# caofff/GL-ABC-MCMC

Measured on AMD Instinct MI355X. Metric: MH accept-steps/sec (whole node) + ESJD, 65 536 chains, Mixture_set dim=2, higher is better.
Workload: dtype f32; 1 GPU; GLMCMC iSIR N=5 gf=0.9, Mixture_set eps=0.05 d=2 (BASELINE configs[1]); chains_per_gpu=65536, batch_size=5, history=True, math_mode=exact, lanes_per_chain=auto, parallelism=chains sharded over 1 GPU(s), no data-path collective

## Files before the change

gl-abc-mcmc_amd/csrc/glabc_device.h:

```cpp
#pragma once

#if !defined(__HIPCC_RTC__)
#include <hip/hip_runtime.h>
#include <stdint.h>
#endif

#include "../../include/glabc.h"
#include "../../include/glabc_numerics.h"

namespace glabc {

#define GLABC_DEV static __device__ __forceinline__

enum Algo { ALGO_GLMCMC = 0, ALGO_GLOBAL = 1 };

enum Variant { VAR_GENERIC = 0, VAR_GAUSS_UNIT = 1, VAR_TAPE = 2, VAR_GAMMA = 3, VAR_MIX = 4 };

template <int D>
struct DistArgs {
    int32_t kind;
    int32_t unit_scale;
    float c0;
    float p0[D], p1[D], p2[D];
    float p3[D];
// ... 256 lines not shown
        const double lp = glabc_gamma_log_pdf((double)g.p0[q], (double)g.p2[q], (double)g.p3[q], z);
#pragma unroll
        for (int r = 0; r < D; ++r) {
            if (r == q) {
                th[r] = (float)z;
                t[r] = lp;
            }
        }
    }
    lq = (float)aten_rowsum_f64<D>(t);
}

template <int D>
GLABC_DEV double mix_mode_term(const MixArgs<D>& m, int k, const double (&z)[D])
{
    double t[D];
#pragma unroll
    for (int q = 0; q < D; ++q) {
        const double e = (z[q] - m.loc[k][q]) * m.inv_scale[k][q];
        t[q] = e * e;
    }
    return glabc_mix_term(m.c0 + m.log_weight[k], aten_rowsum_f64<D>(t), m.sum_log_scale[k]);
}

template <int D>
GLABC_DEV double mix_log_prob(const MixArgs<D>& m, const double (&z)[D])
{
    const int K = m.n_modes;
    double mx = -__builtin_inf();
#pragma unroll 1
    for (int k = 0; k < K; ++k) {
        const double t = mix_mode_term<D>(m, k, z);
        mx = t > mx ? t : mx;
    }
    if (mx == -__builtin_inf() || mx == __builtin_inf()) mx = 0.0;
    double a0 = 0.0, a1 = 0.0, a2 = 0.0, a3 = 0.0, tail = 0.0;
#pragma unroll 1
    for (int k = 0; k < K; ++k) {
        const double e = glabc_exp(mix_mode_term<D>(m, k, z) - mx);
        if (k < 4) {
            a0 = k == 0 ? e : a0;
            a1 = k == 1 ? e : a1;
            a2 = k == 2 ? e : a2;
            a3 = k == 3 ? e : a3;
        } else if (K == 8) {
            a0 = k == 4 ? a0 + e : a0;
            a1 = k == 5 ? a1 + e : a1;
            a2 = k == 6 ? a2 + e : a2;
            a3 = k == 7 ? a3 + e : a3;
        } else {
            tail = tail + e;
        }
    }
    double s;
    if (K < 4) {
        s = a0;
        if (K > 1) s = s + a1;
        if (K > 2) s = s + a2;
    } else {
        s = (((tail + a0) + a1) + a2) + a3;
    }
    return mx + glabc_log(s);
}

template <int D>
GLABC_DEV float dist_mix_log_prob(const MixArgs<D>& m, const float (&z)[D])
{
    double zd[D];
#pragma unroll
    for (int q = 0; q < D; ++q) zd[q] = (double)z[q];
    return (float)mix_log_prob<D>(m, zd);
}

template <int D>
GLABC_DEV void mix_draw(const MixArgs<D>& m, double u, const float (&eps)[D], double (&z)[D])
{
    double sc[D], lc[D];
#pragma unroll
    for (int q = 0; q < D; ++q) {
        sc[q] = m.scale[0][q];
        lc[q] = m.loc[0][q];
    }
#pragma unroll 1
    for (int k = 1; k < m.n_modes; ++k) {
        const bool up = !(u < m.cum_weight[k - 1]);
#pragma unroll
        for (int q = 0; q < D; ++q) {
            sc[q] = up ? m.scale[k][q] : sc[q];
            lc[q] = up ? m.loc[k][q] : lc[q];
        }
    }
#pragma unroll
    for (int q = 0; q < D; ++q) z[q] = (double)eps[q] * sc[q] + lc[q];
}

template <int D>
GLABC_DEV void dist_mix_forward(const MixArgs<D>& m, uint32_t c0, uint32_t c1, uint32_t k0, uint32_t k1, uint32_t step, int j,
                                const float (&eps)[D], float (&th)[D], float& lq)
{
    const glabc_u32x4 w = glabc_philox4x32_10(c0, c1, step, GLABC_SLOT_MIX + (uint32_t)j, k0, k1);
    double z[D];
    mix_draw<D>(m, glabc_uniform_f64(w.v[0], w.v[1]), eps, z);
#pragma unroll
    for (int q = 0; q < D; ++q) th[q] = (float)z[q];
    lq = (float)mix_log_prob<D>(m, z);
}

template <int D, bool KNOWN_GAUSS_UNIT = false, bool GAMMA_OK = false>
GLABC_DEV float dist_log_prob(const DistArgs<D>& g, const float (&z)[D])
{
    if constexpr (GAMMA_OK) {
        if (g.kind == GLABC_DIST_GAMMA) return dist_log_prob_gamma<D>(g, z);
    }
    if (KNOWN_GAUSS_UNIT || g.kind == GLABC_DIST_DIAG_GAUSS) {
        float t[D];
        if (KNOWN_GAUSS_UNIT || g.unit_scale) {
#pragma unroll
            for (int j = 0; j < D; ++j) {
                float e = z[j] - g.p0[j];
                t[j] = 0.5f * (e * e);
            }
        } else {
#pragma unroll
            for (int j = 0; j < D; ++j) {
                float e = (z[j] - g.p0[j]) / g.p2[j];
                t[j] = g.p1[j] + 0.5f * (e * e);
            }
        }
        return g.c0 - aten_rowsum<D>(t);
    } else {
        bool out = false;
#pragma unroll
        for (int j = 0; j < D; ++j) out = out || (z[j] < g.p0[j]) || (z[j] > g.p1[j]);
        return out ? -__builtin_inff() : g.c0;
    }
}

template <int D, bool KNOWN_GAUSS_UNIT = false>
GLABC_DEV float dist_forward_log_p(const DistArgs<D>& g, const float (&noise)[D])
{
    if (KNOWN_GAUSS_UNIT || g.kind == GLABC_DIST_DIAG_GAUSS) {
        float t[D];
#pragma unroll
        for (int j = 0; j < D; ++j) {
            const float h = 0.5f * (noise[j] * noise[j]);
            t[j] = KNOWN_GAUSS_UNIT ? h : g.p1[j] + h;
        }
        return g.c0 - aten_rowsum<D>(t);
    }
    return g.c0;
}

GLABC_DEV float gk_tanhf(float x)
{
    const float e = glabc_expf_core(__builtin_fmaxf(-2.0f * __builtin_fabsf(x), -104.0f));
    const float r = (1.0f - e) / (1.0f + e);
    return x < 0.0f ? -r : r;
}

template <int N>
GLABC_DEV void sort_ascending(float (&v)[N])
{
#pragma unroll
    for (int pass = 0; pass < N; ++pass) {
#pragma unroll
        for (int i = pass & 1; i + 1 < N; i += 2) {
            const float lo = __builtin_fminf(v[i], v[i + 1]), hi = __builtin_fmaxf(v[i], v[i + 1]);
            v[i] = lo;
            v[i + 1] = hi;
        }
    }
}

#ifdef GLABC_USER_SIM
template <int YD> struct NoiseDim { static constexpr int value = GLABC_USER_NOISE_DIM; };
#else
template <int YD> struct NoiseDim { static constexpr int value = YD; };
#endif

template <int D, int YD>
GLABC_DEV void model_simulate(const StepArgs<D, YD>& a, const float (&theta)[D], const float (&eps)[NoiseDim<YD>::value],
                              float (&y)[YD])
{
#ifdef GLABC_USER_SIM
    glabc_user_simulate(theta, eps, y);
    return;
#else
    if constexpr (YD == D) {
        if (D < 4 || a.sim_kind == GLABC_SIM_ABS_GAUSS) {
#pragma unroll
            for (int j = 0; j < YD; ++j) {
                float noise = a.noise_loc[j] + a.noise_scale[j] * eps[j];
                y[j] = __builtin_fabsf(theta[j]) + noise;
            }
            return;
        }
    }
    if constexpr (D >= 4) {
#pragma unroll
        for (int j = 0; j < YD; ++j) {
            const float z = eps[j];
            const float t = gk_tanhf((theta[2] * z) * 0.5f);
            const float pw = glabc_expf(theta[3] * glabc_logf_normal(1.0f + z * z));
            y[j] = theta[0] + ((theta[1] * (1.0f + a.gk_c * t)) * pw) * z;
        }
        sort_ascending<YD>(y);
    }
#endif
}

template <int YD>
GLABC_DEV float model_discrepancy_rows(const float (&y)[YD], const float* y_obs)
{
#ifdef GLABC_USER_DISCREPANCY
    float yo[YD];
#pragma unroll
    for (int j = 0; j < YD; ++j) yo[j] = y_obs[j];
    return glabc_user_discrepancy(y, yo);
#else
    float t[YD];
#pragma unroll
    for (int j = 0; j < YD; ++j) {
        float d = y[j] - y_obs[j];
        t[j] = d * d;
    }
    return __builtin_sqrtf(aten_rowsum<YD>(t));
#endif
}

GLABC_DEV float model_log_kernel_of(float dis, float kern_scale, float kern_log_scale, float kern_c0)
{
#ifdef GLABC_USER_KERNEL
    (void)kern_log_scale;
    (void)kern_c0;
    return glabc_user_log_kernel(dis, kern_scale);
#else
    const float e = (dis - 0.0f) / kern_scale;
    return kern_c0 - (kern_log_scale + 0.5f * (e * e));
#endif
}

template <int D, int YD, bool LEAN_SQRT = false, bool FAST = false>
GLABC_DEV float model_log_kernel(const StepArgs<D, YD>& a, const float (&y)[YD])
{
#if defined(GLABC_USER_DISCREPANCY) || defined(GLABC_USER_KERNEL)
    return model_log_kernel_of(model_discrepancy_rows<YD>(y, a.y_obs), a.kern_scale, a.kern_log_scale, a.kern_c0);
#else
    float t[YD];
#pragma unroll
    for (int j = 0; j < YD; ++j) {
        float d = y[j] - a.y_obs[j];
        t[j] = d * d;
    }
    const float ss = aten_rowsum<YD>(t);
    if constexpr (FAST) {
        const float e = __builtin_amdgcn_sqrtf(ss) * __builtin_amdgcn_rcpf(a.kern_scale);
        return a.kern_c0 - (a.kern_log_scale + 0.5f * (e * e));
    }
    float dis = LEAN_SQRT ? glabc_sqrtf_normal(ss) : __builtin_sqrtf(ss);
    float e;
    if constexpr (LEAN_SQRT) {
        const float q = dis * a.kern_rinv;
        e = __builtin_fmaf(__builtin_fmaf(-q, a.kern_scale, dis), a.kern_rinv, q);
    } else {
        e = (dis - 0.0f) / a.kern_scale;
    }
    return a.kern_c0 - (a.kern_log_scale + 0.5f * (e * e));
#endif
}

template <int D, int YD, bool GU, bool GM>
GLABC_DEV float model_prior(const StepArgs<D, YD>& a, const float (&theta)[D])
{
#ifdef GLABC_USER_PRIOR
    return glabc_user_prior_log_prob(theta);
#else
    return dist_log_prob<D, GU, GM>(a.prior, theta);
#endif
}

struct Rng {
    uint32_t c0, c1, k0, k1;
};

GLABC_DEV void fast_normal_pair(uint32_t a, uint32_t b, float* z0, float* z1)
{
    const float u1 = glabc_uniform_pos_f32(a);
    const float rad = __builtin_amdgcn_sqrtf(-1.3862943611198906f * __builtin_amdgcn_logf(u1));
    const float u2 = glabc_uniform_f32(b);
    *z0 = rad * __builtin_amdgcn_cosf(u2);
    *z1 = rad * __builtin_amdgcn_sinf(u2);
}
GLABC_DEV float fast_expf(float x)
{
    const float t = x * 1.4426950408889634f;
    const bool tiny = t < -126.0f;
    const float r = __builtin_amdgcn_exp2f(tiny ? t + 64.0f : t);
    return tiny ? r * 0x1p-64f : r;
}
GLABC_DEV float fast_logf(float x) { return 0.6931471805599453f * __builtin_amdgcn_logf(x); }

#if defined(__HIPCC_RTC__)
constexpr bool kFastPassWeights = false;
#else
constexpr bool kFastPassWeights = true;
#endif
GLABC_DEV float isir_weight(float lw)
{
    const float v = glabc_expf(lw);
    return (v != v) ? 0.0f : v;
}
GLABC_DEV float isir_weight_approx(float lw)
{
    const float x = __builtin_fminf(__builtin_fmaxf(lw, -104.0f), 100.0f);
    const float t = __builtin_fmaf(x, 0x1.715476p+0f, 12582912.0f);
    const float k = t - 12582912.0f;
    float r = __builtin_fmaf(k, -0x1.62e4p-1f, x);
    r = __builtin_fmaf(k, -0x1.7f7d1cp-20f, r);
    return __builtin_ldexpf(__builtin_amdgcn_exp2f(r * 0x1.715476p+0f), (int)k);
}

template <int L, int SRC>
GLABC_DEV int group_bcast_i(int v)
{
    if constexpr (L == 1) {
        return v;
    } else if constexpr (L == 2) {
        constexpr int ctrl = SRC | (SRC << 2) | ((2 + SRC) << 4) | ((2 + SRC) << 6);
        return __builtin_amdgcn_mov_dpp(v, ctrl, 0xf, 0xf, true);
    } else {
        static_assert(L == 4, "lane groups are 1, 2 or 4 wide");
        constexpr int ctrl = SRC | (SRC << 2) | (SRC << 4) | (SRC << 6);
        return __builtin_amdgcn_mov_dpp(v, ctrl, 0xf, 0xf, true);
    }
}

template <int L, int SRC>
GLABC_DEV float group_bcast(float v)
{
    return __builtin_bit_cast(float, group_bcast_i<L, SRC>(__builtin_bit_cast(int, v)));
}

template <int L>
GLABC_DEV float group_get_dyn(float v, int src)
{
    if constexpr (L == 1) {
        return v;
    } else {
        const int lane = (int)(threadIdx.x & 63u);
        return __shfl(v, (lane & ~(L - 1)) | src, 64);
    }
}

template <int L, int K, int NL>
GLABC_DEV float gather_weight(const float (&wl)[NL])
{
    return group_bcast<L, (K - 1) % L>(wl[(K - 1) / L]);
}

template <int L, int N, int NL, int K = 1>
GLABC_DEV void gather_weights(const float (&wl)[NL], float (&w)[N + 1])
{
    if constexpr (K <= N) {
        w[K] = gather_weight<L, K, NL>(wl);
        gather_weights<L, N, NL, K + 1>(wl, w);
    }
}

template <int D, int YD = D>
struct Chain {
    float theta[D];
    float y[YD];
    float prior;
    float kern;
    float q;
    float log_w;
    float lw_cur;
    float w_cur;
    float gf;
    uint32_t flags;
    uint32_t n_moves;
};

template <int D, int YD, bool GAMMA_OK = false>
GLABC_DEV void refresh_cache(const StepArgs<D, YD>& a, Chain<D, YD>& c)
{
    c.prior = model_prior<D, YD, false, GAMMA_OK>(a, c.theta);
    c.kern = model_log_kernel<D, YD>(a, c.y);
    c.q = dist_log_prob<D, false, GAMMA_OK>(a.global, c.theta);
}

template <int ALGO, int D, int YD, int N, int L, int VAR>
GLABC_DEV bool chain_step(const typename KernelArgs<D, YD, VAR>::type& a, const Rng& rng, uint32_t step, int sub, Chain<D, YD>& c, int64_t tape_pos)
{
    constexpr bool GU = (VAR == VAR_GAUSS_UNIT);
    constexpr bool TAPE = (VAR == VAR_TAPE);
    constexpr bool GM = (VAR == VAR_GAMMA);
    constexpr bool MX = (VAR == VAR_MIX);
    static_assert(!TAPE || L == 1, "tape replay runs one lane per chain");
    static_assert(!GM || L == 1, "the Gamma variant runs one lane per chain");
    static_assert(!MX || L == 1, "the mixture variant runs one lane per chain");
    constexpr int NL = (N + L - 1) / L;
    constexpr int HEAD = L - 1;
    constexpr bool FREE_SLOT = (L > 1) && (N % L != 0) && (NL >= 2);
    constexpr int DP = D + (D & 1);
    constexpr int ND = NoiseDim<YD>::value;
    constexpr int M = DP + ND;
    constexpr int SPP = (M + 3) / 4;

    uint32_t hw[4];
    float log_u = 0.0f;
    bool is_global = false;
    auto take_head = [&]() {
        if constexpr (L > 1) {
#pragma unroll
            for (int q = 0; q < 4; ++q) hw[q] = (uint32_t)group_bcast_i<L, HEAD>((int)hw[q]);
        }
        const float ub = TAPE ? a.tape_u[2 * tape_pos] : glabc_uniform_f32(hw[0]);
        const float ua = TAPE ? a.tape_u[2 * tape_pos + 1] : glabc_uniform_f32(hw[1]);
        log_u = TAPE ? glabc_logf(ua) : ((ua == 0.0f) ? -__builtin_inff() : glabc_logf_normal(ua));
        is_global = ub < c.gf;
        if (ALGO == ALGO_GLMCMC && is_global) {
            if (c.flags & GLABC_FLAG_LOCAL) c.log_w = c.lw_cur;
            c.flags &= ~GLABC_FLAG_LOCAL;
        }
    };
    if constexpr (!FREE_SLOT) {
        if (L == 1 || sub == HEAD) {
            glabc_u32x4 h = glabc_philox4x32_10(rng.c0, rng.c1, step, 0u, rng.k0, rng.k1);
#pragma unroll
            for (int q = 0; q < 4; ++q) hw[q] = h.v[q];
        } else {
#pragma unroll
            for (int q = 0; q < 4; ++q) hw[q] = 0u;
        }
        take_head();
    }

    [[maybe_unused]] float* mix_stage = nullptr;
    if constexpr (MX) {
        static_assert(D <= 4, "the mixture variant is instantiated up to theta_dim 4");
        __shared__ float mix_lds[N * (D + 1) * 64];
        mix_stage = mix_lds + (threadIdx.x & 63u);
#pragma unroll 1
        for (int j = 0; j < N; ++j) {
            const glabc_u32x4 o = glabc_philox4x32_10(rng.c0, rng.c1, step, (uint32_t)(1 + j * SPP), rng.k0, rng.k1);
            float nj[4], ej[D], tm[D], lqm;
            glabc_normal_pair(o.v[0], o.v[1], &nj[0], &nj[1]);
            if constexpr (D > 2) glabc_normal_pair(o.v[2], o.v[3], &nj[2], &nj[3]);
#pragma unroll
            for (int q = 0; q < D; ++q) ej[q] = nj[q];
            dist_mix_forward<D>(mix_of(a), rng.c0, rng.c1, rng.k0, rng.k1, step, j, ej, tm, lqm);
#pragma unroll
            for (int q = 0; q < D; ++q) mix_stage[(j * (D + 1) + q) * 64] = tm[q];
            mix_stage[(j * (D + 1) + D) * 64] = lqm;
        }
    }

    float th[NL][D], yy[NL][YD], lw[NL], pr[NL], kk[NL], wl[NL];
    bool acc_mh = false;
    const bool g_uni = !GU && a.global.kind == GLABC_DIST_UNIFORM;
    const bool l_uni = !GU && a.local.kind == GLABC_DIST_UNIFORM;
#pragma unroll
    for (int rr = 0; rr < NL; ++rr) {
        const int r = FREE_SLOT ? (NL - 1 - rr) : rr;
        const int j = sub + L * r;
        const bool head_pass = FREE_SLOT && (r == NL - 1);
        const bool first = (r == 0) && (L == 1 || sub == 0);
        uint32_t w[4 * SPP];
#pragma unroll
        for (int b = 0; b < SPP; ++b) {
            uint32_t slot_id = (uint32_t)(1 + j * SPP + b);
            if (head_pass && b == 0) slot_id = (sub == HEAD) ? 0u : slot_id;
            glabc_u32x4 o = glabc_philox4x32_10(rng.c0, rng.c1, step, slot_id, rng.k0, rng.k1);
#pragma unroll
            for (int q = 0; q < 4; ++q) w[4 * b + q] = o.v[q];
        }
        if (head_pass) {
#pragma unroll
            for (int q = 0; q < 4; ++q) hw[q] = w[q];
            take_head();
        }
        const bool loc = first && !is_global;
        const bool uni = loc ? l_uni : g_uni;
        float nrm[2 * ((M + 1) / 2)], e[D], s[ND];
#pragma unroll
        for (int i = 0; 2 * i < M; ++i) glabc_normal_pair(w[2 * i], w[2 * i + 1], &nrm[2 * i], &nrm[2 * i + 1]);
#pragma unroll
        for (int i = 0; i < D; ++i) e[i] = (!GU && uni) ? glabc_uniform_f32(w[i]) : nrm[i];
#pragma unroll
        for (int i = 0; i < ND; ++i) s[i] = nrm[DP + i];
        if constexpr (TAPE) {
            const float* tz = a.tape_z + (tape_pos * a.tape_nprop + (j < a.tape_nprop ? j : 0)) * (D + YD);
#pragma unroll
            for (int i = 0; i < D; ++i) e[i] = tz[i];
#pragma unroll
            for (int i = 0; i < ND; ++i) s[i] = tz[D + i];
        }
#pragma unroll
        for (int q = 0; q < D; ++q) {
            const float p0 = loc ? a.local.p0[q] : a.global.p0[q];
            const float p2 = loc ? a.local.p2[q] : a.global.p2[q];
            const float t = p0 + p2 * e[q];
            th[r][q] = loc ? (t + c.theta[q]) : t;
        }
        float lq_gamma = 0.0f;
        const bool g_gam = GM && a.global.kind == GLABC_DIST_GAMMA;
        if constexpr (GM) {
            if (g_gam) {
                float tg[D];
                dist_gamma_forward<D>(a.global, rng.c0, rng.c1, rng.k0, rng.k1, step, j, tg, lq_gamma);
#pragma unroll
                for (int q = 0; q < D; ++q) th[r][q] = loc ? th[r][q] : tg[q];
            }
        }
        float lq_mix = 0.0f;
        if constexpr (MX) {
            lq_mix = mix_stage[(r * (D + 1) + D) * 64];
#pragma unroll
            for (int q = 0; q < D; ++q) th[r][q] = loc ? th[r][q] : mix_stage[(r * (D + 1) + q) * 64];
        }
        float lq;
        if constexpr (MX) {
            lq = lq_mix;
            if constexpr (ALGO == ALGO_GLMCMC) {
                if (loc) lq = dist_mix_log_prob<D>(mix_of(a), th[r]);
            }
        } else if constexpr (ALGO == ALGO_GLMCMC && GU) {
            float v[D];
#pragma unroll
            for (int q = 0; q < D; ++q) v[q] = loc ? (th[r][q] - a.global.p0[q]) : e[q];
            lq = dist_forward_log_p<D, GU>(a.global, v);
        } else if constexpr (ALGO == ALGO_GLMCMC) {
            lq = loc ? dist_log_prob<D, GU, GM>(a.global, th[r]) : (g_gam ? lq_gamma : dist_forward_log_p<D, GU>(a.global, e));
        } else {
            lq = g_gam ? lq_gamma : dist_forward_log_p<D, GU>(a.global, e);
        }
        model_simulate<D, YD>(a, th[r], s, yy[r]);
        pr[r] = model_prior<D, YD, GU, GM>(a, th[r]);
        kk[r] = model_log_kernel<D, YD, GU>(a, yy[r]);
        const float pk = pr[r] + kk[r];
        lw[r] = pk - lq;
        if (r == 0) {
            float log_acc;
            if (ALGO == ALGO_GLOBAL)
                log_acc = loc ? ((pk - c.prior) - c.kern)
                              : ((((pk + c.q) - lq) - c.prior) - c.kern);
            else
                log_acc = (pk - c.prior) - c.kern;
            acc_mh = log_u < log_acc;
        }
        if (ALGO == ALGO_GLMCMC)
            wl[r] = kFastPassWeights ? isir_weight_approx(lw[r]) : isir_weight(lw[r]);
    }

    int ind;
    if constexpr (ALGO == ALGO_GLMCMC) {
        float w[N + 1];
        w[0] = c.w_cur;
        gather_weights<L, N, NL>(wl, w);
        float tot = aten_rowsum<N + 1>(w);
        const double u_res = TAPE ? a.tape_r[tape_pos] : glabc_uniform_f64(hw[2], hw[3]);
        int ig = -1;
        bool sure = !a.exact_index;
        {
            const float rinv = __builtin_amdgcn_rcpf(tot);
            const float u32 = (float)u_res;
            float run = 0.0f;
#pragma unroll
            for (int k = 0; k <= N; ++k) {
                run += w[k] * rinv;
                const float gap = u32 - run;
                sure = sure && (__builtin_fabsf(gap) > 4e-6f);
                ig = (ig < 0 && gap < 0.0f) ? k : ig;
            }
            sure = sure && (run > 0.999f) && (run < 1.001f);
            if constexpr (kFastPassWeights) sure = sure && (tot >= 0x1p-100f) && (tot < 0x1p126f);
        }
        if (!sure) {
            if constexpr (kFastPassWeights) {
                float lwg[N + 1];
                gather_weights<L, N, NL>(lw, lwg);
#pragma unroll
                for (int k = 1; k <= N; ++k) w[k] = isir_weight(lwg[k]);
                tot = aten_rowsum<N + 1>(w);
            }
            ig = -1;
            double run = 0.0;
#pragma unroll
            for (int k = 0; k <= N; ++k) {
                run += (double)(w[k] / tot);
                ig = (ig < 0 && u_res < run) ? k : ig;
            }
        }
        ig = ig < 0 ? 0 : ig;
        const int il = group_bcast_i<L, 0>(acc_mh ? 1 : 0);
        ind = is_global ? ig : il;
    } else {
        ind = group_bcast_i<L, 0>(acc_mh ? 1 : 0);
    }

    const bool moved = ind > 0;
    if (__any(moved)) {
        const int owner = (ind - 1) & (L - 1);
        const int slot = (ind - 1) / L;
        constexpr bool CARRY_W = (ALGO == ALGO_GLMCMC) && !kFastPassWeights;
        float nt[D], ny[YD], nlw = lw[0], npr = pr[0], nkk = kk[0], nw = CARRY_W ? wl[0] : 0.0f;
#pragma unroll
// ... 58 lines not shown
```

gl-abc-mcmc_amd/csrc/glabc_geometry.h:

```cpp
#pragma once

#include "../../include/glabc.h"

namespace glabc {


constexpr int team_main_candidates(int n, int nw)
{
    const int t10 = (10 * n + 11) / nw - 11;
    const int na = (t10 + 5) / 10;
    return na < 1 ? 1 : (na > n - (nw - 1) ? n - (nw - 1) : na);
}
constexpr int team_helper_first(int n, int nw, int h)
{
    const int na = team_main_candidates(n, nw), nh = n - na, per = nh / (nw - 1), extra = nh % (nw - 1);
    return na + h * per + (h < extra ? h : extra);
}
constexpr bool team_split_ok(int n, int nw) { return n >= nw && team_main_candidates(n, nw) >= 1; }

constexpr int team_lds_bytes(int d, int yd, int n, int nw) { return 2 * (n - team_main_candidates(n, nw)) * (4 + d + yd) * 64 * 4; }
constexpr int TEAM_MAX_LDS = 40 * 1024;
constexpr bool team_config_ok(int d, int yd, int n, int nw)
{
    return n >= 2 && n <= GLABC_MAX_BATCH && team_split_ok(n, nw) && team_lds_bytes(d, yd, n, nw) <= TEAM_MAX_LDS;
}

constexpr int GLOBAL_TEAM_CHUNK = 8;
constexpr int global_team_lds_bytes(int d, int nd) { return 2 * GLOBAL_TEAM_CHUNK * (2 + d + 2 * ((nd + 1) / 2)) * 64 * 4; }


constexpr int WIDE_BLOCK = 256;
constexpr int WIDE_LANES[4] = {8, 16, 32, 64};
constexpr int wide_default_lanes(int n) { return n <= 64 ? 8 : n <= 128 ? 16 : n <= 256 ? 32 : 64; }
constexpr int wide_row_floats(int n) { return n + 1 + 32; }
constexpr int64_t wide_lds_bytes(int l, int n) { return (int64_t)4 * (WIDE_BLOCK / l) * wide_row_floats(n); }


constexpr int pick_lanes(int requested, int n_batch, int64_t n_chains)
{
    int lanes = requested;
    if (lanes <= 0) {
        const int64_t chip_lanes = 64 * 1024;
        lanes = 1;
        while (lanes < 4 && n_chains * lanes < chip_lanes) lanes *= 2;
    }
    if (lanes >= 4 && n_batch >= 3) return 4;
    if (lanes >= 2 && n_batch >= 2) return 2;
    return 1;
}

}
```

gl-abc-mcmc_amd/csrc/glabc_team.h:

```cpp
#pragma once

#include "glabc_device.h"
#include "glabc_geometry.h"

namespace glabc {

template <int D, int YD, int NH>
struct TeamCand {
    float wl[NH][64];
    float lw[NH][64];
    float pr[NH][64];
    float kk[NH][64];
    float th[NH][D][64];
    float yy[NH][YD][64];
};

template <int D, int YD, int VAR, bool FIRST, bool FAST = false>
GLABC_DEV void team_candidate(const StepArgs<D, YD>& a, const Rng& rng, uint32_t step, int j, bool loc, const Chain<D, YD>& c,
                              float (&th)[D], float (&yy)[YD], float& lw, float& pr, float& kk, float& wl, int64_t row = 0,
                              int n_prop = 0, bool dump = false)
{
    constexpr bool GU = (VAR == VAR_GAUSS_UNIT);
    constexpr bool GM = (VAR == VAR_GAMMA);
    constexpr int DP = D + (D & 1);
    constexpr int ND = NoiseDim<YD>::value;
    constexpr int M = DP + ND;
    constexpr int SPP = (M + 3) / 4;
    const bool g_uni = !GU && a.global.kind == GLABC_DIST_UNIFORM;
    const bool l_uni = !GU && a.local.kind == GLABC_DIST_UNIFORM;
    uint32_t w[4 * SPP];
#pragma unroll
    for (int b = 0; b < SPP; ++b) {
        glabc_u32x4 o = glabc_philox4x32_10(rng.c0, rng.c1, step, (uint32_t)(1 + j * SPP + b), rng.k0, rng.k1);
#pragma unroll
        for (int q = 0; q < 4; ++q) w[4 * b + q] = o.v[q];
    }
    const bool lc = FIRST && loc;
    const bool uni = lc ? l_uni : g_uni;
    float nrm[2 * ((M + 1) / 2)], e[D], s[ND];
#pragma unroll
    for (int i = 0; 2 * i < M; ++i) {
        if constexpr (FAST) fast_normal_pair(w[2 * i], w[2 * i + 1], &nrm[2 * i], &nrm[2 * i + 1]);
        else glabc_normal_pair(w[2 * i], w[2 * i + 1], &nrm[2 * i], &nrm[2 * i + 1]);
    }
#pragma unroll
    for (int i = 0; i < D; ++i) e[i] = (!GU && uni) ? glabc_uniform_f32(w[i]) : nrm[i];
#pragma unroll
    for (int i = 0; i < ND; ++i) s[i] = nrm[DP + i];
    if constexpr (FAST) {
        if (dump) {
            float* z = a.dump_z + (row * n_prop + j) * (D + ND);
#pragma unroll
            for (int i = 0; i < D; ++i) z[i] = e[i];
#pragma unroll
            for (int i = 0; i < ND; ++i) z[D + i] = s[i];
        }
    }
#pragma unroll
    for (int q = 0; q < D; ++q) {
        const float p0 = lc ? a.local.p0[q] : a.global.p0[q];
        const float p2 = lc ? a.local.p2[q] : a.global.p2[q];
        const float t = (GU && !FIRST) ? p0 + e[q] : p0 + p2 * e[q];
        th[q] = lc ? (t + c.theta[q]) : t;
    }
    float lq_gamma = 0.0f;
    const bool g_gam = GM && a.global.kind == GLABC_DIST_GAMMA;
    if constexpr (GM) {
        if (g_gam) {
            float tg[D];
            dist_gamma_forward<D>(a.global, rng.c0, rng.c1, rng.k0, rng.k1, step, j, tg, lq_gamma);
#pragma unroll
            for (int q = 0; q < D; ++q) th[q] = lc ? th[q] : tg[q];
        }
    }
    float lq;
    if constexpr (GU) {
        float v[D];
#pragma unroll
        for (int q = 0; q < D; ++q) v[q] = lc ? (th[q] - a.global.p0[q]) : e[q];
        lq = dist_forward_log_p<D, GU>(a.global, v);
    } else {
        lq = lc ? dist_log_prob<D, GU, GM>(a.global, th) : (g_gam ? lq_gamma : dist_forward_log_p<D, GU>(a.global, e));
    }
    model_simulate<D, YD>(a, th, s, yy);
    pr = model_prior<D, YD, GU, GM>(a, th);
    kk = model_log_kernel<D, YD, GU, FAST>(a, yy);
    lw = (pr + kk) - lq;
    if constexpr (FAST) {
        const float v = fast_expf(lw);
        wl = (v != v) ? 0.0f : v;
    } else {
        wl = kFastPassWeights ? isir_weight_approx(lw) : isir_weight(lw);
    }
}

template <int D, int YD, int N, int VAR, int NA, int LO, int HI, bool FAST>
GLABC_DEV void team_helper(const StepArgs<D, YD>& a, const Rng& rng, int lane, TeamCand<D, YD, N - NA> (&buf)[2], int64_t chain, bool valid)
{
    Chain<D, YD> none;
#pragma unroll 1
    for (int t = 0; t < a.n_steps; ++t) {
        const uint32_t step = a.step0 + (uint32_t)t;
        TeamCand<D, YD, N - NA>& o = buf[t & 1];
#pragma unroll
        for (int j = LO; j < HI; ++j) {
            float th[D], yy[YD], lw, pr, kk, wl;
            team_candidate<D, YD, VAR, false, FAST>(a, rng, step, j, false, none, th, yy, lw, pr, kk, wl,
                                                    chain * (int64_t)a.n_steps + t, N, FAST && valid && a.dump_z != nullptr);
            o.wl[j - NA][lane] = wl;
            o.lw[j - NA][lane] = lw;
            o.pr[j - NA][lane] = pr;
            o.kk[j - NA][lane] = kk;
#pragma unroll
            for (int q = 0; q < D; ++q) o.th[j - NA][q][lane] = th[q];
#pragma unroll
            for (int q = 0; q < YD; ++q) o.yy[j - NA][q][lane] = yy[q];
        }
        __syncthreads();
    }
}

template <int D, int YD, int N, int VAR, int NW, bool FAST = false>
__global__ void __launch_bounds__(64 * NW) __attribute__((amdgpu_waves_per_eu(NW))) team_sampler_kernel(const StepArgs<D, YD> a, int prio)
{
    constexpr bool GU = (VAR == VAR_GAUSS_UNIT);
    constexpr bool GM = (VAR == VAR_GAMMA);
    static_assert(NW >= 2 && NW <= 4 && team_split_ok(N, NW), "team of two to four wavefronts, at least one candidate each");
    constexpr int NA = team_main_candidates(N, NW), NH = N - NA;
    __shared__ TeamCand<D, YD, NH> buf[2];
    const int wave = (int)(threadIdx.x >> 6), lane = (int)(threadIdx.x & 63u);
    const int64_t tid = (int64_t)blockIdx.x * 64 + lane;
    const bool valid = tid < a.n_chains;
    const int64_t i = valid ? tid : a.n_chains - 1;
    const uint64_t gid = (uint64_t)(a.chain0 + i);
    Rng rng;
    rng.c0 = (uint32_t)gid;
    rng.c1 = (uint32_t)(gid >> 32);
    rng.k0 = a.seed_lo;
    rng.k1 = a.seed_hi;

    if (wave != 0) {
        if (wave == 1) team_helper<D, YD, N, VAR, NA, team_helper_first(N, NW, 0), team_helper_first(N, NW, 1), FAST>(a, rng, lane, buf, i, valid);
        if constexpr (NW >= 3) {
            if (wave == 2) team_helper<D, YD, N, VAR, NA, team_helper_first(N, NW, 1), team_helper_first(N, NW, 2), FAST>(a, rng, lane, buf, i, valid);
        }
        if constexpr (NW >= 4) {
            if (wave == 3) team_helper<D, YD, N, VAR, NA, team_helper_first(N, NW, 2), team_helper_first(N, NW, 3), FAST>(a, rng, lane, buf, i, valid);
        }
        return;
    }

    if (prio == 1) __builtin_amdgcn_s_setprio(1);
    else if (prio == 2) __builtin_amdgcn_s_setprio(2);
    else if (prio == 3) __builtin_amdgcn_s_setprio(3);
    Chain<D, YD> c;
#pragma unroll
    for (int j = 0; j < D; ++j) c.theta[j] = a.theta[j * a.stride + i];
#pragma unroll
    for (int j = 0; j < YD; ++j) c.y[j] = a.y[j * a.stride + i];
    c.log_w = a.log_w[i];
    c.flags = a.flags[i];
    c.n_moves = a.n_moves ? a.n_moves[i] : 0u;
    c.gf = a.gf_chain ? a.gf_chain[i] : a.gf;
    refresh_cache<D, YD, GM>(a, c);
    if constexpr (FAST) c.kern = model_log_kernel<D, YD, false, true>(a, c.y);
    c.lw_cur = (c.flags & GLABC_FLAG_LOCAL) ? (c.prior + c.kern) - c.q : c.log_w;
    {
        const float v = FAST ? fast_expf(c.lw_cur) : glabc_expf(c.lw_cur);
        c.w_cur = (v != v) ? 0.0f : v;
    }
    constexpr int TRI = D * (D + 1) / 2;
    const bool mom = a.sum_theta != nullptr;
    double s1[D], s2[TRI], sj[TRI];
    if (mom) {
#pragma unroll
        for (int j = 0; j < D; ++j) s1[j] = a.sum_theta[j * a.stride + i];
#pragma unroll
        for (int k = 0; k < TRI; ++k) {
            s2[k] = a.sum_outer[k * a.stride + i];
            sj[k] = a.sum_jump[k * a.stride + i];
        }
    }
    float* hist = a.history ? a.history + i : nullptr;

#pragma unroll 1
    for (int t = 0; t < a.n_steps; ++t) {
        const uint32_t step = a.step0 + (uint32_t)t;
        float prev[D];
#pragma unroll
        for (int j = 0; j < D; ++j) prev[j] = c.theta[j];

        glabc_u32x4 hd = glabc_philox4x32_10(rng.c0, rng.c1, step, 0u, rng.k0, rng.k1);
        const float ub = glabc_uniform_f32(hd.v[0]), ua = glabc_uniform_f32(hd.v[1]);
        const float log_u = FAST ? fast_logf(ua) : ((ua == 0.0f) ? -__builtin_inff() : glabc_logf_normal(ua));
        const bool is_global = ub < c.gf;
        const int64_t row = i * (int64_t)a.n_steps + t;
        const bool dump = FAST && valid && a.dump_z != nullptr;
        if constexpr (FAST) {
            if (dump) {
                a.dump_u[2 * row] = ub;
                a.dump_u[2 * row + 1] = ua;
                a.dump_r[row] = glabc_uniform_f64(hd.v[2], hd.v[3]);
            }
        }
        if (is_global) {
            if (c.flags & GLABC_FLAG_LOCAL) c.log_w = c.lw_cur;
            c.flags &= ~GLABC_FLAG_LOCAL;
        }
        float th[NA][D], yy[NA][YD], lw[NA], pr[NA], kk[NA], wl[NA];
        team_candidate<D, YD, VAR, true, FAST>(a, rng, step, 0, !is_global, c, th[0], yy[0], lw[0], pr[0], kk[0], wl[0], row, N, dump);
        const bool acc_mh = log_u < (((pr[0] + kk[0]) - c.prior) - c.kern);
#pragma unroll
        for (int r = 1; r < NA; ++r)
            team_candidate<D, YD, VAR, false, FAST>(a, rng, step, r, false, c, th[r], yy[r], lw[r], pr[r], kk[r], wl[r], row, N, dump);

        __syncthreads();
        const TeamCand<D, YD, NH>& in = buf[t & 1];

        float w[N + 1];
        w[0] = c.w_cur;
#pragma unroll
        for (int r = 0; r < NA; ++r) w[1 + r] = wl[r];
#pragma unroll
        for (int r = 0; r < NH; ++r) w[1 + NA + r] = in.wl[r][lane];
        float tot = aten_rowsum<N + 1>(w);
        const double u_res = glabc_uniform_f64(hd.v[2], hd.v[3]);
        int ig = -1;
        bool sure = !a.exact_index;
        {
            const float rinv = __builtin_amdgcn_rcpf(tot);
            const float u32 = (float)u_res;
            float run = 0.0f;
#pragma unroll
            for (int k = 0; k <= N; ++k) {
                run += w[k] * rinv;
                const float gap = u32 - run;
                sure = sure && (__builtin_fabsf(gap) > 4e-6f);
                ig = (ig < 0 && gap < 0.0f) ? k : ig;
            }
            sure = sure && (run > 0.999f) && (run < 1.001f);
            if constexpr (!FAST && kFastPassWeights) sure = sure && (tot >= 0x1p-100f) && (tot < 0x1p126f);
        }
        if (!sure) {
            if constexpr (!FAST && kFastPassWeights) {
#pragma unroll
                for (int r = 0; r < NA; ++r) w[1 + r] = isir_weight(lw[r]);
#pragma unroll
                for (int r = 0; r < NH; ++r) w[1 + NA + r] = isir_weight(in.lw[r][lane]);
                tot = aten_rowsum<N + 1>(w);
            }
            ig = -1;
            double run = 0.0;
#pragma unroll
            for (int k = 0; k <= N; ++k) {
                run += (double)(w[k] / tot);
                ig = (ig < 0 && u_res < run) ? k : ig;
            }
        }
        ig = ig < 0 ? 0 : ig;
        const int ind = is_global ? ig : (acc_mh ? 1 : 0);

        const bool moved = ind > 0;
        if (__any(moved)) {
            float nt[D], ny[YD], nlw = lw[0], npr = pr[0], nkk = kk[0], nw = wl[0];
#pragma unroll
            for (int q = 0; q < D; ++q) nt[q] = th[0][q];
#pragma unroll
            for (int q = 0; q < YD; ++q) ny[q] = yy[0][q];
#pragma unroll
            for (int r = 1; r < NA; ++r) {
                if (ind - 1 == r) {
#pragma unroll
                    for (int q = 0; q < D; ++q) nt[q] = th[r][q];
#pragma unroll
                    for (int q = 0; q < YD; ++q) ny[q] = yy[r][q];
                    nlw = lw[r];
                    npr = pr[r];
                    nkk = kk[r];
                    nw = wl[r];
                }
            }
            if (ind - 1 >= NA) {
                const int r = ind - 1 - NA;
#pragma unroll
                for (int q = 0; q < D; ++q) nt[q] = in.th[r][q][lane];
#pragma unroll
                for (int q = 0; q < YD; ++q) ny[q] = in.yy[r][q][lane];
                nlw = in.lw[r][lane];
                npr = in.pr[r][lane];
                nkk = in.kk[r][lane];
                nw = in.wl[r][lane];
            }
            if (moved) {
#pragma unroll
                for (int q = 0; q < D; ++q) c.theta[q] = nt[q];
#pragma unroll
                for (int q = 0; q < YD; ++q) c.y[q] = ny[q];
                c.prior = npr;
                c.kern = nkk;
                c.q = dist_log_prob<D, GU, GM>(a.global, c.theta);
                c.lw_cur = nlw;
                c.w_cur = (FAST || !kFastPassWeights) ? nw : isir_weight(nlw);
                if (is_global)
                    c.log_w = nlw;
                else
                    c.flags |= GLABC_FLAG_LOCAL;
            }
        }
        c.n_moves += moved ? 1u : 0u;

        if (hist && valid) {
#pragma unroll
            for (int j = 0; j < D; ++j) hist[((int64_t)t * D + j) * a.hist_stride] = c.theta[j];
        }
        if (mom) {
            int k = 0;
#pragma unroll
            for (int p = 0; p < D; ++p) {
                s1[p] += (double)c.theta[p];
#pragma unroll
                for (int q = p; q < D; ++q, ++k) {
                    s2[k] = glabc_add_prod_f32(s2[k], c.theta[p], c.theta[q]);
                    double dp = (double)c.theta[p] - (double)prev[p];
                    double dq = (double)c.theta[q] - (double)prev[q];
                    sj[k] += dp * dq;
                }
            }
        }
    }

    if (valid) {
#pragma unroll
        for (int j = 0; j < D; ++j) a.theta[j * a.stride + i] = c.theta[j];
#pragma unroll
        for (int j = 0; j < YD; ++j) a.y[j * a.stride + i] = c.y[j];
        a.log_w[i] = c.log_w;
        a.flags[i] = c.flags;
        if (a.n_moves) a.n_moves[i] = c.n_moves;
        if (mom) {
#pragma unroll
            for (int j = 0; j < D; ++j) a.sum_theta[j * a.stride + i] = s1[j];
#pragma unroll
            for (int k = 0; k < TRI; ++k) {
                a.sum_outer[k * a.stride + i] = s2[k];
                a.sum_jump[k * a.stride + i] = sj[k];
            }
        }
    }
}

template <int D, int YD>
struct GlobalDraws {
    float log_u[64];
    uint32_t is_global[64];
    float e[D][64];
    uint32_t sw[2 * ((NoiseDim<YD>::value + 1) / 2)][64];
};

template <int D, int YD, int VAR, int NW>
__global__ void __launch_bounds__(64 * NW) __attribute__((amdgpu_waves_per_eu(NW))) global_team_kernel(const StepArgs<D, YD> a, int prio)
{
    static_assert(NW == 2 || NW == 3, "a team of two or three wavefronts");
    constexpr bool GU = (VAR == VAR_GAUSS_UNIT);
    constexpr int DP = D + (D & 1);
    constexpr int ND = NoiseDim<YD>::value;
    constexpr int M = DP + ND;
    constexpr int SPP = (M + 3) / 4;
    constexpr int CH = GLOBAL_TEAM_CHUNK;
    __shared__ GlobalDraws<D, YD> buf[2][CH];
    const int wave = (int)(threadIdx.x >> 6), lane = (int)(threadIdx.x & 63u);
    const int64_t tid = (int64_t)blockIdx.x * 64 + lane;
    const bool valid = tid < a.n_chains;
    const int64_t i = valid ? tid : a.n_chains - 1;
    const uint64_t gid = (uint64_t)(a.chain0 + i);
    Rng rng;
    rng.c0 = (uint32_t)gid;
    rng.c1 = (uint32_t)(gid >> 32);
    rng.k0 = a.seed_lo;
    rng.k1 = a.seed_hi;
    const float gf = a.gf_chain ? a.gf_chain[i] : a.gf;

    if (wave != 0) {
        const bool g_uni = !GU && a.global.kind == GLABC_DIST_UNIFORM;
        const bool l_uni = !GU && a.local.kind == GLABC_DIST_UNIFORM;
        const bool do_head = NW == 2 || wave == 1, do_cand = NW == 2 || wave == 2;
        const bool need_branch = do_head || g_uni != l_uni;
#pragma unroll 1
        for (int t0 = 0; t0 < a.n_steps; t0 += CH) {
#pragma unroll 1
          for (int t = t0; t < t0 + CH && t < a.n_steps; ++t) {
            const uint32_t step = a.step0 + (uint32_t)t;
            GlobalDraws<D, YD>& o = buf[(t0 / CH) & 1][t - t0];
            bool is_global = false;
            if (need_branch) {
                const glabc_u32x4 h = glabc_philox4x32_10(rng.c0, rng.c1, step, 0u, rng.k0, rng.k1);
                const float ub = glabc_uniform_f32(h.v[0]);
                is_global = ub < gf;
                if (do_head) {
                    const float ua = glabc_uniform_f32(h.v[1]);
                    o.log_u[lane] = (ua == 0.0f) ? -__builtin_inff() : glabc_logf_normal(ua);
                    o.is_global[lane] = is_global ? 1u : 0u;
                }
            }
            if (do_cand) {
                uint32_t w[4 * SPP];
#pragma unroll
                for (int b = 0; b < SPP; ++b) {
                    const glabc_u32x4 v = glabc_philox4x32_10(rng.c0, rng.c1, step, (uint32_t)(1 + b), rng.k0, rng.k1);
#pragma unroll
                    for (int q = 0; q < 4; ++q) w[4 * b + q] = v.v[q];
                }
                const bool uni = is_global ? g_uni : l_uni;
                float nrm[DP];
#pragma unroll
                for (int k = 0; 2 * k < DP; ++k) glabc_normal_pair(w[2 * k], w[2 * k + 1], &nrm[2 * k], &nrm[2 * k + 1]);
#pragma unroll
                for (int k = 0; k < D; ++k) o.e[k][lane] = (!GU && uni) ? glabc_uniform_f32(w[k]) : nrm[k];
#pragma unroll
                for (int k = 0; k < 2 * ((ND + 1) / 2); ++k) o.sw[k][lane] = w[DP + k];
            }
          }
            __syncthreads();
        }
        return;
    }

    if (prio == 1) __builtin_amdgcn_s_setprio(1);
    Chain<D, YD> c;
#pragma unroll
    for (int j = 0; j < D; ++j) c.theta[j] = a.theta[j * a.stride + i];
#pragma unroll
    for (int j = 0; j < YD; ++j) c.y[j] = a.y[j * a.stride + i];
    c.log_w = 0.0f;
    c.flags = 0u;
    c.n_moves = a.n_moves ? a.n_moves[i] : 0u;
    c.gf = gf;
    refresh_cache<D, YD>(a, c);
    constexpr int TRI = D * (D + 1) / 2;
    const bool mom = a.sum_theta != nullptr;
    double s1[D], s2[TRI], sj[TRI];
    if (mom) {
#pragma unroll
        for (int j = 0; j < D; ++j) s1[j] = a.sum_theta[j * a.stride + i];
#pragma unroll
        for (int k = 0; k < TRI; ++k) {
            s2[k] = a.sum_outer[k * a.stride + i];
            sj[k] = a.sum_jump[k * a.stride + i];
        }
    }
    float* hist = a.history ? a.history + i : nullptr;

#pragma unroll 1
    for (int t0 = 0; t0 < a.n_steps; t0 += CH) {
      __syncthreads();
#pragma unroll 1
      for (int t = t0; t < t0 + CH && t < a.n_steps; ++t) {
        float prev[D];
#pragma unroll
        for (int j = 0; j < D; ++j) prev[j] = c.theta[j];
        const GlobalDraws<D, YD>& in = buf[(t0 / CH) & 1][t - t0];
        const float log_u = in.log_u[lane];
        const bool is_global = in.is_global[lane] != 0u;
        float e[D], sn[ND];
#pragma unroll
        for (int k = 0; k < D; ++k) e[k] = in.e[k][lane];
        {
            float nn[2 * ((ND + 1) / 2)];
#pragma unroll
            for (int k = 0; 2 * k < ND; ++k) glabc_normal_pair(in.sw[2 * k][lane], in.sw[2 * k + 1][lane], &nn[2 * k], &nn[2 * k + 1]);
#pragma unroll
            for (int k = 0; k < ND; ++k) sn[k] = nn[k];
        }
        const bool loc = !is_global;
        float th[D], yy[YD];
#pragma unroll
        for (int q = 0; q < D; ++q) {
            const float p0 = loc ? a.local.p0[q] : a.global.p0[q];
            const float p2 = loc ? a.local.p2[q] : a.global.p2[q];
            const float tt = p0 + p2 * e[q];
            th[q] = loc ? (tt + c.theta[q]) : tt;
        }
        const float lq = dist_forward_log_p<D, GU>(a.global, e);
        model_simulate<D, YD>(a, th, sn, yy);
        const float pr = model_prior<D, YD, GU, false>(a, th);
        const float kk = model_log_kernel<D, YD, GU>(a, yy);
        const float pk = pr + kk;
        const float log_acc = loc ? ((pk - c.prior) - c.kern)
                                  : ((((pk + c.q) - lq) - c.prior) - c.kern);
        const bool moved = log_u < log_acc;
        if (moved) {
#pragma unroll
            for (int q = 0; q < D; ++q) c.theta[q] = th[q];
#pragma unroll
            for (int q = 0; q < YD; ++q) c.y[q] = yy[q];
            c.prior = pr;
            c.kern = kk;
            c.q = dist_log_prob<D, GU>(a.global, c.theta);
        }
        c.n_moves += moved ? 1u : 0u;
        if (hist && valid) {
#pragma unroll
            for (int j = 0; j < D; ++j) hist[((int64_t)t * D + j) * a.hist_stride] = c.theta[j];
        }
        if (mom) {
            int k = 0;
#pragma unroll
            for (int p = 0; p < D; ++p) {
                s1[p] += (double)c.theta[p];
#pragma unroll
                for (int q = p; q < D; ++q, ++k) {
                    s2[k] = glabc_add_prod_f32(s2[k], c.theta[p], c.theta[q]);
                    double dp = (double)c.theta[p] - (double)prev[p];
                    double dq = (double)c.theta[q] - (double)prev[q];
                    sj[k] += dp * dq;
                }
            }
        }
      }
    }
    if (valid) {
#pragma unroll
        for (int j = 0; j < D; ++j) a.theta[j * a.stride + i] = c.theta[j];
#pragma unroll
        for (int j = 0; j < YD; ++j) a.y[j * a.stride + i] = c.y[j];
        if (a.n_moves) a.n_moves[i] = c.n_moves;
        if (mom) {
#pragma unroll
            for (int j = 0; j < D; ++j) a.sum_theta[j * a.stride + i] = s1[j];
#pragma unroll
            for (int k = 0; k < TRI; ++k) {
                a.sum_outer[k * a.stride + i] = s2[k];
                a.sum_jump[k * a.stride + i] = sj[k];
            }
        }
    }
}

#if !defined(__HIPCC_RTC__)
template <int D, int YD>
int launch_team_dim(int n_batch, int nw, const StepArgs<D, YD>& a, int prio, bool fast, hipStream_t stream);
template <int D, int YD>
int launch_global_team_dim(int nw, const StepArgs<D, YD>& a, int prio, hipStream_t stream);
#endif

}
```

Baseline: 35.51 billion chain-steps/s.

## Offload per-step moment and jump accumulation from main wave to helper waves

The main wavefront of the team sampler no longer updates the fp64 running sums (theta, outer product, jump) each step. It writes its current theta into a small double-buffered LDS trace. Helper waves read that trace two steps later, accumulate the sums, and write them back at the end; the split is gated by whether the extra LDS keeps CU occupancy unchanged. The aim is to take serial fp64 arithmetic off the main wave's critical path, at the cost of extra LDS traffic, an extra barrier and more helper register pressure.

```diff
diff --git a/gl-abc-mcmc_amd/csrc/glabc_device.h b/gl-abc-mcmc_amd/csrc/glabc_device.h
--- a/gl-abc-mcmc_amd/csrc/glabc_device.h
+++ b/gl-abc-mcmc_amd/csrc/glabc_device.h
@@ -582,8 +582,10 @@
 
 #if defined(__HIPCC_RTC__)
 constexpr bool kFastPassWeights = false;
+constexpr bool kTeamHelperSums = false;
 #else
 constexpr bool kFastPassWeights = true;
+constexpr bool kTeamHelperSums = true;
 #endif
 GLABC_DEV float isir_weight(float lw)
 {
diff --git a/gl-abc-mcmc_amd/csrc/glabc_geometry.h b/gl-abc-mcmc_amd/csrc/glabc_geometry.h
--- a/gl-abc-mcmc_amd/csrc/glabc_geometry.h
+++ b/gl-abc-mcmc_amd/csrc/glabc_geometry.h
@@ -25,6 +25,20 @@
     return n >= 2 && n <= GLABC_MAX_BATCH && team_split_ok(n, nw) && team_lds_bytes(d, yd, n, nw) <= TEAM_MAX_LDS;
 }
 
+constexpr int TEAM_CU_LDS = 160 * 1024, TEAM_CU_WORKGROUPS = 8;
+constexpr int team_trace_bytes(int d) { return 2 * d * 64 * 4; }
+constexpr int team_cu_workgroups(int lds, int granule)
+{
+    const int fit = (TEAM_CU_LDS / granule) / ((lds + granule - 1) / granule);
+    return fit > TEAM_CU_WORKGROUPS ? TEAM_CU_WORKGROUPS : fit;
+}
+constexpr bool team_trace_fits(int d, int yd, int n, int nw)
+{
+    const int lds = team_lds_bytes(d, yd, n, nw), with = lds + team_trace_bytes(d);
+    return team_cu_workgroups(with, 1) == team_cu_workgroups(lds, 1) && team_cu_workgroups(with, 512) == team_cu_workgroups(lds, 512) &&
+           team_cu_workgroups(with, 1280) == team_cu_workgroups(lds, 1280);
+}
+
 constexpr int GLOBAL_TEAM_CHUNK = 8;
 constexpr int global_team_lds_bytes(int d, int nd) { return 2 * GLOBAL_TEAM_CHUNK * (2 + d + 2 * ((nd + 1) / 2)) * 64 * 4; }
 
diff --git a/gl-abc-mcmc_amd/csrc/glabc_team.h b/gl-abc-mcmc_amd/csrc/glabc_team.h
--- a/gl-abc-mcmc_amd/csrc/glabc_team.h
+++ b/gl-abc-mcmc_amd/csrc/glabc_team.h
@@ -94,14 +94,67 @@
     }
 }
 
-template <int D, int YD, int N, int VAR, int NA, int LO, int HI, bool FAST>
-GLABC_DEV void team_helper(const StepArgs<D, YD>& a, const Rng& rng, int lane, TeamCand<D, YD, N - NA> (&buf)[2], int64_t chain, bool valid)
+template <int D>
+struct TeamTrace {
+    float th[2][D][64];
+};
+
+template <int D, int YD, int N, int VAR, int NA, int LO, int HI, bool FAST, bool SUMS, bool S12, bool SJ>
+GLABC_DEV void team_helper(const StepArgs<D, YD>& a, const Rng& rng, int lane, TeamCand<D, YD, N - NA> (&buf)[2], const TeamTrace<D>& trace,
+                           int64_t chain, bool valid)
 {
     Chain<D, YD> none;
+    constexpr int TRI = D * (D + 1) / 2;
+    constexpr bool KEEP = SUMS && (S12 || SJ);
+    const bool mom = KEEP && a.sum_theta != nullptr;
+    double s1[D], s2[TRI], sj[TRI];
+    float prev[D];
+    if constexpr (KEEP) {
+        if (mom) {
+            if constexpr (S12) {
+#pragma unroll
+                for (int j = 0; j < D; ++j) s1[j] = a.sum_theta[j * a.stride + chain];
+#pragma unroll
+                for (int k = 0; k < TRI; ++k) s2[k] = a.sum_outer[k * a.stride + chain];
+            }
+            if constexpr (SJ) {
+#pragma unroll
+                for (int k = 0; k < TRI; ++k) sj[k] = a.sum_jump[k * a.stride + chain];
+#pragma unroll
+                for (int j = 0; j < D; ++j) prev[j] = a.theta[j * a.stride + chain];
+            }
+        }
+    }
+    auto consume = [&](int slot) {
+        float th[D];
+#pragma unroll
+        for (int p = 0; p < D; ++p) th[p] = trace.th[slot][p][lane];
+        int k = 0;
+#pragma unroll
+        for (int p = 0; p < D; ++p) {
+            if constexpr (S12) s1[p] += (double)th[p];
+#pragma unroll
+            for (int q = p; q < D; ++q, ++k) {
+                if constexpr (S12) s2[k] = glabc_add_prod_f32(s2[k], th[p], th[q]);
+                if constexpr (SJ) {
+                    double dp = (double)th[p] - (double)prev[p];
+                    double dq = (double)th[q] - (double)prev[q];
+                    sj[k] += dp * dq;
+                }
+            }
+        }
+        if constexpr (SJ) {
+#pragma unroll
+            for (int p = 0; p < D; ++p) prev[p] = th[p];
+        }
+    };
 #pragma unroll 1
     for (int t = 0; t < a.n_steps; ++t) {
         const uint32_t step = a.step0 + (uint32_t)t;
         TeamCand<D, YD, N - NA>& o = buf[t & 1];
+        if constexpr (KEEP) {
+            if (mom && t >= 2) consume(t & 1);
+        }
 #pragma unroll
         for (int j = LO; j < HI; ++j) {
             float th[D], yy[YD], lw, pr, kk, wl;
@@ -118,6 +171,27 @@
         }
         __syncthreads();
     }
+    if constexpr (SUMS) {
+        __syncthreads();
+        if constexpr (KEEP) {
+            if (mom) {
+#pragma unroll 1
+                for (int t = a.n_steps >= 2 ? a.n_steps - 2 : 0; t < a.n_steps; ++t) consume(t & 1);
+                if (valid) {
+                    if constexpr (S12) {
+#pragma unroll
+                        for (int j = 0; j < D; ++j) a.sum_theta[j * a.stride + chain] = s1[j];
+#pragma unroll
+                        for (int k = 0; k < TRI; ++k) a.sum_outer[k * a.stride + chain] = s2[k];
+                    }
+                    if constexpr (SJ) {
+#pragma unroll
+                        for (int k = 0; k < TRI; ++k) a.sum_jump[k * a.stride + chain] = sj[k];
+                    }
+                }
+            }
+        }
+    }
 }
 
 template <int D, int YD, int N, int VAR, int NW, bool FAST = false>
@@ -127,7 +201,10 @@
     constexpr bool GM = (VAR == VAR_GAMMA);
     static_assert(NW >= 2 && NW <= 4 && team_split_ok(N, NW), "team of two to four wavefronts, at least one candidate each");
     constexpr int NA = team_main_candidates(N, NW), NH = N - NA;
+    constexpr bool SUMS = kTeamHelperSums && team_trace_fits(D, YD, N, NW) && !(GM && D == 4 && YD == 4 && N == 5 && NW == 2);
+    static_assert(sizeof(TeamTrace<D>) == team_trace_bytes(D), "the trace the geometry accounts for");
     __shared__ TeamCand<D, YD, NH> buf[2];
+    __shared__ TeamTrace<D> trace;
     const int wave = (int)(threadIdx.x >> 6), lane = (int)(threadIdx.x & 63u);
     const int64_t tid = (int64_t)blockIdx.x * 64 + lane;
     const bool valid = tid < a.n_chains;
@@ -140,12 +217,12 @@
     rng.k1 = a.seed_hi;
 
     if (wave != 0) {
-        if (wave == 1) team_helper<D, YD, N, VAR, NA, team_helper_first(N, NW, 0), team_helper_first(N, NW, 1), FAST>(a, rng, lane, buf, i, valid);
+        if (wave == 1) team_helper<D, YD, N, VAR, NA, team_helper_first(N, NW, 0), team_helper_first(N, NW, 1), FAST, SUMS, true, NW == 2>(a, rng, lane, buf, trace, i, valid);
         if constexpr (NW >= 3) {
-            if (wave == 2) team_helper<D, YD, N, VAR, NA, team_helper_first(N, NW, 1), team_helper_first(N, NW, 2), FAST>(a, rng, lane, buf, i, valid);
+            if (wave == 2) team_helper<D, YD, N, VAR, NA, team_helper_first(N, NW, 1), team_helper_first(N, NW, 2), FAST, SUMS, false, NW == 3>(a, rng, lane, buf, trace, i, valid);
         }
         if constexpr (NW >= 4) {
-            if (wave == 3) team_helper<D, YD, N, VAR, NA, team_helper_first(N, NW, 2), team_helper_first(N, NW, 3), FAST>(a, rng, lane, buf, i, valid);
+            if (wave == 3) team_helper<D, YD, N, VAR, NA, team_helper_first(N, NW, 2), team_helper_first(N, NW, 3), FAST, SUMS, false, true>(a, rng, lane, buf, trace, i, valid);
         }
         return;
     }
@@ -172,7 +249,7 @@
     constexpr int TRI = D * (D + 1) / 2;
     const bool mom = a.sum_theta != nullptr;
     double s1[D], s2[TRI], sj[TRI];
-    if (mom) {
+    if (!SUMS && mom) {
 #pragma unroll
         for (int j = 0; j < D; ++j) s1[j] = a.sum_theta[j * a.stride + i];
 #pragma unroll
@@ -313,7 +390,11 @@
 #pragma unroll
             for (int j = 0; j < D; ++j) hist[((int64_t)t * D + j) * a.hist_stride] = c.theta[j];
         }
-        if (mom) {
+        if (SUMS && mom) {
+#pragma unroll
+            for (int j = 0; j < D; ++j) trace.th[t & 1][j][lane] = c.theta[j];
+        }
+        if (!SUMS && mom) {
             int k = 0;
 #pragma unroll
             for (int p = 0; p < D; ++p) {
@@ -329,6 +410,7 @@
         }
     }
 
+    if constexpr (SUMS) __syncthreads();
     if (valid) {
 #pragma unroll
         for (int j = 0; j < D; ++j) a.theta[j * a.stride + i] = c.theta[j];
@@ -337,7 +419,7 @@
         a.log_w[i] = c.log_w;
         a.flags[i] = c.flags;
         if (a.n_moves) a.n_moves[i] = c.n_moves;
-        if (mom) {
+        if (!SUMS && mom) {
 #pragma unroll
             for (int j = 0; j < D; ++j) a.sum_theta[j * a.stride + i] = s1[j];
 #pragma unroll
```

Measured after the change: 33.35 billion chain-steps/s. 6.1% lower.
